# atx/padne

Measured on AMD Instinct MI355X. Metric: CG solves/s, higher is better.
Workload: dtype f64; 1 GPU; C4 8-layer N=10M: 8-layer jittered triangular Laplacian, 9999392 nodes, via-ring stitched, 1 A source/sink, amg-PCG to rtol 1e-12; n_unknowns=9999391, nnz_per_rank=69955225, rows_per_rank=9999391, parallelism=layer-partitioned x1

## Files before the change

padne_amd/_hip.py:

```python
from __future__ import annotations

import ctypes as C
import weakref
import os
import sys
from dataclasses import dataclass

import numpy as np

_HERE = os.path.dirname(os.path.abspath(__file__))
LIB_PATH = os.path.join(_HERE, "libpadne_hip.so")

OK = 0
E_INVALID, E_HIP, E_NOMEM, E_NONMANIFOLD, E_NOTCONVERGED, E_COMM, E_BREAKDOWN, E_TOOLARGE, E_NOCOARSEN = \
    -1, -2, -3, -4, -5, -6, -7, -8, -9


class HipUnavailableError(RuntimeError):
    """libpadne_hip.so cannot be loaded or no MI355X is visible."""


class HipError(RuntimeError):
    def __init__(self, code: int, message: str):
        super().__init__(f"libpadne_hip error {code}: {message}")
# ... 80 lines not shown
                                            _PI64, _PF64, _I64, _PI64, _PF64, C.POINTER(SolveOpts), C.c_double,
                                            C.POINTER(SolveInfo)]),
    "padne_kkt_power_density_block": (C.c_int, [_P, _P, C.c_int32, _PF64]),
    "padne_kkt_sensitivity_block": (C.c_int, [_P, _P, C.c_int32, C.c_int32, _PF64, _PF64, _PF64, _PF64]),
    "padne_kkt_current_report": (C.c_int, [_P, _P, C.c_int32, C.c_int64, C.c_int32, _PI32, C.c_int32, _PI32, _PF64, _PF64, _PF64,
                                           _PF64, _PI64, _PF64]),
    "padne_kkt_current_cases": (C.c_int, [_P, _P, C.c_int32, C.c_int64, C.c_int32, _PI32, C.c_int32, _PI32, _PF64, _PF64, _PF64,
                                          _PF64, _PI32, _PF64, _PI64, _PF64, _PF64]),
    "padne_kkt_error_estimate": (C.c_int, [_P, _P, C.c_int32, C.c_int64, C.c_int64, C.c_int32, _PF64, _PF64, _PF64, _PF64, _PF64,
                                           _PI64]),
    "padne_amg_apply": (C.c_int, [_P, _P, _PF64, _PF64]),
    "padne_amg_apply_batch": (C.c_int, [_P, _P, C.c_int32, _PF64, _PF64, _PF64]),
    "padne_csr_set_preconditioner_block": (C.c_int, [_P, _P]),
    "padne_amg_level": (C.c_int, [_P, _P, C.c_int, C.c_int, C.POINTER(_P)]),
    "padne_nearest_vertex": (C.c_int, [_P, _I64, _PF64, _I64, _PF64, _PI64]),
    "padne_nearest_vertex_ties": (C.c_int, [_P, _I64, _PF64, _I64, _PF64, _PI64, _PI32]),
    "padne_power_density": (C.c_int, [_P, _I64, _PF64, _I64, _PI32, _I64, _PI64, _PI64, _PF64, _PF64, _PF64]),
    "padne_csr_power_density": (C.c_int, [_P, _P, _PF64, _PF64]),
    "padne_face_gradient": (C.c_int, [_P, _I64, _PF64, _I64, _PI32, _I64, _PI64, _PI64, _PF64, _PF64, _PF64]),
    "padne_error_estimate": (C.c_int, [_P, _I64, _PF64, _I64, _PI32, _I64, _PI64, _PI64, _PF64, _PF64, _PF64, _PF64, _PF64, _PF64,
                                       _PF64, _PI64]),
    "padne_refine_create": (C.c_int, [_P, _I64, _PF64, _I64, _PI32, _I64, _PI64, _PI64, C.POINTER(C.c_uint8), _PI64, _PI64, _PI64,
                                      C.POINTER(_P)]),
    "padne_refine_fetch": (C.c_int, [_P, _P, _PF64, _PI32, _PI32, _PI32]),
    "padne_refine_destroy": (C.c_int, [_P]),
    "padne_sampler_create": (C.c_int, [_P, _I64, _PF64, _I64, _PI32, C.c_int32, _PI64, _PI64, _PI32, _PF64, C.c_int32, _PF64, _I64,
                                       C.POINTER(_P)]),
    "padne_sampler_destroy": (C.c_int, [_P]),
    "padne_sampler_points": (C.c_int, [_P, _P, C.c_int32, _I64, _PF64, _PI32, _PF64, _PF64, _PF64]),
    "padne_sampler_raster": (C.c_int, [_P, _P, C.c_int32, C.c_double, C.c_double, C.c_double, C.c_double, _I64, _I64, _PI32,
                                       _PF64, _PF64, _PF64]),
    "padne_sampler_stats": (C.c_int, [_P, C.c_int32, _PI64, _PF64]),
    "padne_spmv_algorithmic_bytes": (_I64, [_P]),
    "padne_spmv_time": (C.c_int, [_P, _P, _P, _P, C.c_int, C.c_int, _PF64]),
}

TEST_SIGNATURES = {
    "padne_team_create": (C.c_int, [C.c_int, C.POINTER(_P)]),
    "padne_team_destroy": (C.c_int, [_P]),
    "padne_team_abort": (C.c_int, [_P]),
    "padne_ctx_join_team": (C.c_int, [_P, _P, C.c_int]),
    "padne_csr_split_tiles": (C.c_int, [_P, C.c_int, _PI64, _PI64]),
    "padne_ctx_lockstep_groups": (C.c_int, [_P, _PI64]),
    "padne_asm_second_path_count": (C.c_int, [_PI64]),
    "padne_ctx_halo_exchange_time": (C.c_int, [_P, C.c_int32, C.POINTER(C.c_double)]),
    "padne_ctx_reload_options": (C.c_int, [_P]),
}

PROBE_SIGNATURES = {
    "padne_test_product": (C.c_int, [_P, _P, C.c_int32, _I64, C.c_int32, C.c_int32, C.c_int32, C.c_int32, _P, _P, _P, _P, _P,
                                     _P, _P, _P, _P, C.c_double, _P, _PF64, _I64, _PI32]),
}

_lib = None


def load_library(path: str | None = None) -> C.CDLL:
    global _lib
    if _lib is not None and path is None:
        return _lib
    p = path or LIB_PATH
    if not os.path.exists(p):
        raise HipUnavailableError(
            f"{p} not found: build it with `python -m padne_amd.build` (hipcc --offload-arch=gfx950). "
            "padne_amd has no CPU fallback.")
    if "torch" in sys.modules:
        pass
    try:
        lib = C.CDLL(p, mode=C.RTLD_GLOBAL)
    except OSError as exc:
        raise HipUnavailableError(f"cannot load {p}: {exc}") from exc
    for name, (res, args) in list(SIGNATURES.items()) + list(TEST_SIGNATURES.items()) + list(PROBE_SIGNATURES.items()):
        fn = getattr(lib, name)
        fn.restype = res
        fn.argtypes = args
    if lib.padne_abi_version() != 1:
        raise HipUnavailableError("libpadne_hip.so ABI version mismatch; rebuild it")
    if path is None:
        _lib = lib
    return lib


def _check(rc: int) -> None:
    if rc == OK:
        return
    msg = (load_library().padne_last_error() or b"").decode("utf-8", "replace")
    if rc == E_NONMANIFOLD:
        raise ValueError(msg or "Non-manifold mesh")
    if rc == E_INVALID:
        raise ValueError(msg)
    if rc == E_NOMEM:
        raise MemoryError(msg)
    if rc == E_TOOLARGE:
        raise OverflowError(msg)
    if rc == E_NOTCONVERGED:
        raise NotConvergedError(rc, msg)
    raise HipError(rc, msg)


def _f64(a) -> np.ndarray:
    return np.ascontiguousarray(a, dtype=np.float64)


def _i32(a) -> np.ndarray:
    return np.ascontiguousarray(a, dtype=np.int32)


def _i64(a) -> np.ndarray:
    return np.ascontiguousarray(a, dtype=np.int64)


def _ptr(a: np.ndarray, typ):
    return a.ctypes.data_as(typ)


def device_count() -> int:
    n = load_library().padne_device_count()
    return max(n, 0)


def launch_count() -> int:
    n = C.c_longlong(0)
    _check(load_library().padne_launch_count(C.byref(n)))
    return int(n.value)

# ... 65 lines not shown
        _check(self._lib.padne_ctx_comm_init(self._h, buf, int(rank), int(world_size)))

    def comm_init_host(self, rank: int, world_size: int, allgather):
        world_size = int(world_size)

        def cb(_user, send, recv, nbytes):
            try:
                src = np.ctypeslib.as_array(C.cast(send, C.POINTER(C.c_ubyte)), shape=(int(nbytes),)).copy()
                out = np.frombuffer(allgather(src), dtype=np.uint8)
                if out.size != world_size * int(nbytes):
                    return 2
                C.memmove(recv, out.ctypes.data, out.size)
                return 0
            except BaseException:
                return 1
        self._host_allgather = ALLGATHER_FN(cb)
        _check(self._lib.padne_ctx_comm_init_host(self._h, int(rank), world_size, C.cast(self._host_allgather, _P), None))

    def p2p_export(self, slots_per_rank: int) -> bytes:
        buf = C.create_string_buffer(64)
        _check(self._lib.padne_ctx_p2p_export(self._h, int(slots_per_rank), buf))
        return buf.raw

    def p2p_import(self, handles: bytes, world_size: int) -> None:
        buf = C.create_string_buffer(bytes(handles), 64 * int(world_size))
        _check(self._lib.padne_ctx_p2p_import(self._h, buf, int(world_size)))

    def p2p_selftest(self) -> bool:
        ok = C.c_int32(0)
        _check(self._lib.padne_ctx_p2p_selftest(self._h, C.byref(ok)))
        return bool(ok.value)

    def p2p_close(self) -> None:
        _check(self._lib.padne_ctx_p2p_close(self._h))

    def comm_call_counts(self):
        calls = (C.c_longlong * 4)()
        nbytes = (C.c_longlong * 4)()
        _check(self._lib.padne_comm_call_counts(calls, nbytes))
        return list(calls), list(nbytes)

    def reload_options(self) -> None:
        _check(self._lib.padne_ctx_reload_options(self._h))

    def halo_exchange_time(self, repeats: int = 200) -> float:
        t = C.c_double(0.0)
        _check(self._lib.padne_ctx_halo_exchange_time(self._h, int(repeats), C.byref(t)))
        return float(t.value)

    def lockstep_groups(self) -> int:
        g = C.c_int64(0)
        _check(self._lib.padne_ctx_lockstep_groups(self._h, C.byref(g)))
        return int(g.value)

    def set_halo(self, n_owned: int, m: int, export_idx) -> None:
        e = _i32(export_idx)
        _check(self._lib.padne_ctx_set_halo(self._h, int(n_owned), int(m), int(e.shape[0]), _ptr(e, _PI32)))
        self.halo_n_owned = int(n_owned)

    def clear_halo(self) -> None:
        _check(self._lib.padne_ctx_set_halo(self._h, -1, 0, 0, None))
        self.halo_n_owned = None

    def alloc(self, nbytes: int) -> int:
        p = _P()
        _check(self._lib.padne_dev_alloc(self._h, int(nbytes), C.byref(p)))
        return int(p.value)

    def free(self, dev: int):
        _check(self._lib.padne_dev_free(self._h, _P(dev)))

    def upload(self, dev: int, host: np.ndarray):
        host = np.ascontiguousarray(host)
        _check(self._lib.padne_dev_upload(self._h, _P(dev), host.ctypes.data_as(_P), host.nbytes))

    def download(self, dev: int, shape, dtype=np.float64) -> np.ndarray:
        out = np.empty(shape, dtype=dtype)
        _check(self._lib.padne_dev_download(self._h, out.ctypes.data_as(_P), _P(dev), out.nbytes))
        return out

    def to_device(self, host: np.ndarray) -> "DeviceArray":
        host = np.ascontiguousarray(host)
        d = DeviceArray(self, host.shape, host.dtype)
        self.upload(d.ptr, host)
        return d

    def empty(self, shape, dtype=np.float64) -> "DeviceArray":
        return DeviceArray(self, shape, dtype)

    def csr_from_scipy(self, A) -> "CsrMatrix":
        import scipy.sparse as sp
        A = sp.csr_matrix(A)
        A.sum_duplicates()
        A.sort_indices()
        if A.nnz >= 2**31 - 8192:
            raise ValueError("matrix too large for int32 indices")
        indptr, indices, data = _i32(A.indptr), _i32(A.indices), _f64(A.data)
        h = _P()
        _check(self._lib.padne_csr_from_host(self._h, A.shape[0], A.shape[1], _ptr(indptr, _PI32),
                                             _ptr(indices, _PI32), _ptr(data, _PF64), C.byref(h)))
        return CsrMatrix(self, h)

    def assemble_system(self, n_unknowns, xy, tri, mesh_vertex_offset, mesh_tri_offset, conductance,
                        coo_row, coo_col, coo_val, partial_mesh: bool = False) -> "CsrMatrix":
        xy_dev = isinstance(xy, DeviceArray)
        tri_dev = isinstance(tri, DeviceArray)
# ... 695 lines not shown
```

padne_amd/build.py:

```python
from __future__ import annotations

import os
import shutil
import subprocess
import sys

HERE = os.path.dirname(os.path.abspath(__file__))
CSRC = os.path.join(HERE, "csrc")
LIB = os.path.join(HERE, "libpadne_hip.so")
SOURCES = ["capi.hip", "spmv.hip", "spmm.hip", "pcg.hip", "assemble.hip", "comm.hip", "amg.hip", "generate.hip", "kkt.hip", "sample.hip", "error.hip", "refine.hip"]
HEADERS = ["common.hpp", "face.hpp", os.path.join("..", "..", "include", "padne_hip.h"),
           os.path.join("..", "..", "include", "padne_hip_test.h"), os.path.join("..", "..", "include", "padne_hip_probe.h")]
ARCH = "gfx950"
FLAGS = ["-O3", "-std=c++17", "-fPIC", f"--offload-arch={ARCH}", "-ffp-contract=off",
         "-fno-fast-math", "-Wall", "-Wno-unused-function", "-Wno-unused-value", "-Wno-unused-result"]


def hipcc() -> str:
    exe = shutil.which("hipcc") or "/opt/rocm/bin/hipcc"
    if not os.path.exists(exe):
        raise RuntimeError("hipcc not found: libpadne_hip.so cannot be built")
    return exe


def needs_build() -> bool:
    if not os.path.exists(LIB):
        return True
    t = os.path.getmtime(LIB)
    deps = [os.path.join(CSRC, s) for s in SOURCES + HEADERS] + [os.path.abspath(__file__)]
    return any(os.path.getmtime(d) > t for d in deps)


def build(force: bool = False, verbose: bool = True) -> str:
    if not force and not needs_build():
        return LIB
    objs = []
    cc = hipcc()
    os.makedirs(os.path.join(CSRC, "build"), exist_ok=True)
    procs = []
    for src in SOURCES:
        obj = os.path.join(CSRC, "build", src.replace(".hip", ".o"))
        cmd = [cc, *FLAGS, "-c", os.path.join(CSRC, src), "-o", obj]
        if verbose:
            print(" ".join(cmd), flush=True)
        procs.append((src, subprocess.Popen(cmd)))
        objs.append(obj)
    for src, p in procs:
        if p.wait() != 0:
            raise RuntimeError(f"hipcc failed on {src}")
    cmd = [cc, "-shared", "-fPIC", f"--offload-arch={ARCH}", "-o", LIB, *objs, "-ldl",
           "-Wl,-rpath,/opt/rocm/lib"]
    if verbose:
        print(" ".join(cmd), flush=True)
    subprocess.check_call(cmd)
    return LIB


if __name__ == "__main__":
    build(force="--force" in sys.argv)
    print(LIB)
```

padne_amd/csrc/assemble.hip:

```cpp
#include "common.hpp"
#include "face.hpp"

#include <atomic>

#include <cmath>

#include <algorithm>

#include <string.h>

namespace padne {

constexpr int kScanItems = 16;
constexpr int kScanChunk = 256 * kScanItems;

__device__ __forceinline__ int block_exclusive_scan_256(int v, int *lds , int *total) {
    const int lane = threadIdx.x & 63, w = threadIdx.x >> 6;
    int inc = v;
#pragma unroll
    for (int off = 1; off < 64; off <<= 1) {
        const int t = __shfl_up(inc, off, 64);
        if (lane >= off) inc += t;
    }
    if (lane == 63) lds[w] = inc;
// ... 115 lines not shown
    }
    if (blockIdx.x == 0 && threadIdx.x == 0) out[n] = (int)(*total);
}

constexpr int kScanSmall = 32768;
__global__ __launch_bounds__(1024) void scan_small(const int *in, const int n, int *out,
                                                   long long *__restrict__ total_out, unsigned long long *mail_slot,
                                                   unsigned long long mail_seq) {
    __shared__ long long wave_tot[16];
    __shared__ int any_neg;
    const int t = threadIdx.x, lane = t & 63, w = t >> 6;
    if (t == 0) any_neg = 0;
    __syncthreads();
    const int per = (n + 1023) / 1024;
    const int b0 = min(t * per, n), b1 = min(b0 + per, n);
    long long s = 0;
    bool neg = false;
    for (int i = b0; i < b1; ++i) {
        const int v = in[i];
        neg |= v < 0;
        s += v;
    }
    if (neg) any_neg = 1;
    long long inc = s;
#pragma unroll
    for (int off = 1; off < 64; off <<= 1) {
        const long long u = __shfl_up(inc, off, 64);
        if (lane >= off) inc += u;
    }
    if (lane == 63) wave_tot[w] = inc;
    __syncthreads();
    long long run = inc - s, total = 0;
    for (int q = 0; q < 16; ++q) {
        if (q < w) run += wave_tot[q];
        total += wave_tot[q];
    }
    for (int i = b0; i < b1; ++i) {
        const int v = in[i];
        out[i] = (int)run;
        run += v;
    }
    if (t == 0) {
        const long long tot = any_neg ? 0 : total;
        out[n] = (int)tot;
        total_out[0] = tot;
        total_out[1] = any_neg;
        if (mail_slot != nullptr) {
            const unsigned long long wd[2] = {(unsigned long long)tot, (unsigned long long)any_neg};
            mail_post(mail_slot, mail_seq, wd, 2);
        }
    }
}

int scan_i32_begin(padne_ctx *ctx, const int32_t *in, int32_t *out, int64_t n, ScanTicket *t, bool want_total) {
    const int nb = (int)((n + kScanChunk - 1) / kScanChunk);
    hipStream_t s = ctx->stream;
    t->nb = nb;
    t->bs = nullptr;
    t->want_total = want_total;
    t->mail = MailTicket();
    if (nb == 0) {
        const hipError_t e = hipMemsetAsync(out, 0, sizeof(int32_t), s);
        if (e != hipSuccess) {
            set_error("scan failed: %s", hipGetErrorString(e));
            return PADNE_E_HIP;
        }
        return PADNE_OK;
    }
    long long *bs = (long long *)pool_alloc(ctx, sizeof(long long) * (size_t)(nb + 2));
    if (bs == nullptr) return PADNE_E_NOMEM;
    t->bs = bs;
    long long *tot = bs + nb;
    if (want_total) t->mail = mail_ticket(ctx);
    if (n <= kScanSmall) {
        hipLaunchKernelGGL(scan_small, dim3(1), dim3(1024), 0, s, in, (int)n, out, tot, t->mail.slot_dev, t->mail.seq);
    } else {
        hipLaunchKernelGGL(scan_block_sums, dim3(nb), dim3(256), 0, s, in, (long long)n, bs);
        hipLaunchKernelGGL(scan_block_offsets, dim3(1), dim3(256), 0, s, bs, nb, tot, t->mail.slot_dev, t->mail.seq);
        hipLaunchKernelGGL(scan_apply, dim3(nb), dim3(256), 0, s, in, (long long)n, bs, tot, out);
    }
    const hipError_t e = hipGetLastError();
    if (e != hipSuccess) {
        pool_free(ctx, bs);
        t->bs = nullptr;
        set_error("scan failed: %s", hipGetErrorString(e));
        return PADNE_E_HIP;
    }
    return PADNE_OK;
}

int scan_i32_end(padne_ctx *ctx, ScanTicket *t, long long h[2]) {
    h[0] = h[1] = 0;
    if (t->nb == 0) return PADNE_OK;
    hipStream_t s = ctx->stream;
    long long *tot = t->bs + t->nb;
    hipError_t e = hipSuccess;
    int rc = PADNE_OK;
    if (t->want_total) {
        if (t->mail.slot_dev != nullptr) {
            rc = mail_wait(ctx, t->mail, h, 2 * sizeof(long long));
        } else {
            e = hipMemcpyAsync(h, tot, 2 * sizeof(long long), hipMemcpyDeviceToHost, s);
            if (e == hipSuccess) e = hipStreamSynchronize(s);
        }
    }
    pool_free(ctx, t->bs);
    t->bs = nullptr;
    if (e != hipSuccess) {
        set_error("scan failed: %s", hipGetErrorString(e));
        return PADNE_E_HIP;
    }
    return rc;
}

static int scan_i32_impl(padne_ctx *ctx, const int32_t *in, int32_t *out, int64_t n, long long h[2], bool want_total) {
    ScanTicket t;
    PADNE_TRY(scan_i32_begin(ctx, in, out, n, &t, want_total));
    return scan_i32_end(ctx, &t, h);
}

int exclusive_scan_i32(padne_ctx *ctx, const int32_t *in, int32_t *out, int64_t n, int64_t *total) {
    long long h[2] = {0, 0};
    PADNE_TRY(scan_i32_impl(ctx, in, out, n, h, true));
    if (h[0] < 0 || h[1] != 0) {
        set_error("scan of negative counts");
        return PADNE_E_INVALID;
    }
    if (h[0] >= 2147483647LL) {
// ... 256 lines not shown
    const bool fc = hubs_of == nullptr || hubs_of[gc] > kIncCap;
    if (!(fa || fb || fc)) return;
    const double ax = xy[2 * (long long)ga], ay = xy[2 * (long long)ga + 1];
    const double bx = xy[2 * (long long)gb], by = xy[2 * (long long)gb + 1];
    const double cx = xy[2 * (long long)gc], cy = xy[2 * (long long)gc + 1];
    const double wab = cot_half(ax, ay, bx, by, cx, cy);
    const double wbc = cot_half(bx, by, cx, cy, ax, ay);
    const double wca = cot_half(cx, cy, ax, ay, bx, by);
    int s;
    if (fa) {
        s = slot_ptr[ga] + atomicAdd(&cursor[ga], 2);
        key[s] = make_key(gb, 0); val[s] = wab;
        key[s + 1] = make_key(gc, 1); val[s + 1] = wca;
    }
    if (fb) {
        s = slot_ptr[gb] + atomicAdd(&cursor[gb], 2);
        key[s] = make_key(gc, 0); val[s] = wbc;
        key[s + 1] = make_key(ga, 1); val[s + 1] = wab;
    }
    if (fc) {
        s = slot_ptr[gc] + atomicAdd(&cursor[gc], 2);
        key[s] = make_key(ga, 0); val[s] = wca;
        key[s + 1] = make_key(gb, 1); val[s + 1] = wbc;
    }
}

__global__ __launch_bounds__(256) void asm_fill_listed(const int *__restrict__ n_list, const int *__restrict__ row_list,
                                                       long long n_vert, const double *__restrict__ xy,
                                                       const int *__restrict__ n_inc, const int2 *__restrict__ inc,
                                                       const int *__restrict__ slot_ptr, int *__restrict__ cursor,
                                                       long long *__restrict__ key, double *__restrict__ val) {
    const int idx = blockIdx.x * blockDim.x + threadIdx.x;
    if (idx >= *n_list) return;
    const int r = row_list[idx];
    const int T = r < n_vert ? n_inc[r] : 0;
    if (T > kIncCap) {
        cursor[r] = 1;
        return;
    }
    cursor[r] = 1 + 2 * T;
    if (T == 0) return;
    const double2 pv = reinterpret_cast<const double2 *>(xy)[r];
    const int s0 = slot_ptr[r];
    for (int q = 0; q < T; ++q) {
        const int2 jk = inc[inc_at(r, q, n_vert)];
        const double2 pj = reinterpret_cast<const double2 *>(xy)[jk.x], pk = reinterpret_cast<const double2 *>(xy)[jk.y];
        key[s0 + 1 + 2 * q] = make_key(jk.x, 0);
        val[s0 + 1 + 2 * q] = cot_half(pv.x, pv.y, pj.x, pj.y, pk.x, pk.y);
        key[s0 + 2 + 2 * q] = make_key(jk.y, 1);
        val[s0 + 2 + 2 * q] = cot_half(pk.x, pk.y, pv.x, pv.y, pj.x, pj.y);
    }
}

constexpr unsigned long long kScanValueMask = (1ull << 62) - 1ull;
constexpr unsigned long long kScanKnown = 1ull << 62;
constexpr int kScanMaxPolls = 1 << 20;
constexpr int kChunkTiles = 64;
__device__ __forceinline__ unsigned long long scan_word_load(const unsigned long long *p) {
    return __hip_atomic_load(p, __ATOMIC_RELAXED, __HIP_MEMORY_SCOPE_AGENT);
}
__device__ __forceinline__ void scan_word_store(unsigned long long *p, unsigned long long v) {
    __hip_atomic_store(p, v, __ATOMIC_RELAXED, __HIP_MEMORY_SCOPE_AGENT);
}
struct TileScan {
    unsigned long long *tile_agg;
    unsigned long long *chunk_agg;
    unsigned long long *chunk_prefix;
    int *chunk_count;
    int *ticket, *abort_word;
    long long *nnz_out;
    int n_tiles, n_chunks;
};

__device__ __forceinline__ void chunk_offset_scanner(const TileScan sc) {
    const int lane = threadIdx.x & 63;
    long long running = 0;
    int done = 0;
    if (lane == 0) scan_word_store(&sc.chunk_prefix[0], kScanKnown);
    int idle = 0;
    while (done < sc.n_chunks) {
        const int idx = done + lane;
        const unsigned long long w = idx < sc.n_chunks ? scan_word_load(&sc.chunk_agg[idx]) : 0ull;
        const unsigned long long gaps = __ballot((w >> 62) == 0ull);
        const int lead = gaps != 0ull ? __ffsll((long long)gaps) - 1 : 64;
        if (lead == 0) {
            if (++idle > kScanMaxPolls || ((idle & 255) == 0 && __hip_atomic_load(sc.abort_word, __ATOMIC_RELAXED, __HIP_MEMORY_SCOPE_AGENT) != 0)) {
                if (lane == 0) __hip_atomic_store(sc.abort_word, 1, __ATOMIC_RELAXED, __HIP_MEMORY_SCOPE_AGENT);
                return;
            }
            __builtin_amdgcn_s_sleep(2);
            continue;
        }
        idle = 0;
        long long incl = lane < lead ? (long long)(w & kScanValueMask) : 0;
        for (int off = 1; off < 64; off <<= 1) {
            const long long up = __shfl_up(incl, off, 64);
            if (lane >= off) incl += up;
        }
        if (lane < lead) scan_word_store(&sc.chunk_prefix[idx + 1], kScanKnown | (unsigned long long)(running + incl));
        running += __shfl(incl, 63, 64);
        done += lead;
    }
    if (lane == 0) *sc.nnz_out = running;
}

__device__ __forceinline__ int tile_publish(const TileScan sc, const int tile, const int total, const int lane) {
    int arrived = 0;
    if (lane == 0) {
        scan_word_store(&sc.tile_agg[tile], kScanKnown | (unsigned long long)total);
        arrived = __hip_atomic_fetch_add(&sc.chunk_count[tile / kChunkTiles], 1, __ATOMIC_RELAXED, __HIP_MEMORY_SCOPE_AGENT) + 1;
    }
    return arrived;
}
__device__ __forceinline__ bool chunk_publish(const TileScan sc, const int tile, const int arrived_lane0, const int lane) {
    const int c = tile / kChunkTiles;
    const int in_chunk = min(kChunkTiles, sc.n_tiles - c * kChunkTiles);
// ... 2220 lines not shown
                if (rc == PADNE_OK && e == hipSuccess) rc = read_back(ctx, d_err, sizeof(h_err), h_err);
            }
        }
        if (rc == PADNE_OK && e != hipSuccess) {
            set_error("row kernel failed: %s", hipGetErrorString(e));
            rc = PADNE_E_HIP;
        }
        if (rc == PADNE_OK && (h_err[ERR_SCAN] || h_err[ERR_GAVE_UP])) {
            set_error("the rows of the assembled system do not fit their offsets (inconsistent row lengths)");
            rc = PADNE_E_HIP;
        }
        if (rc == PADNE_OK && h_err[ERR_NONMANIFOLD] && !t_partial_mesh) {
            set_error("Non-manifold mesh");
            rc = PADNE_E_NONMANIFOLD;
        }
    } else {
        PADNE_HIP_CHECK(hipMemsetAsync(m->rowptr, 0, sizeof(int32_t), s));
    }
    if (rc == PADNE_OK && (h_nnz < 0 || h_nnz > nnz_bound)) {
        set_error("assembled %lld entries where at most %lld fit", h_nnz, nnz_bound);
        rc = PADNE_E_HIP;
    }
    if (rc == PADNE_OK) {
        rc = csr_shrink_nnz(ctx, m, h_nnz);
        if (rc == PADNE_OK && hipStreamSynchronize(s) != hipSuccess) {
            set_error("assembly failed: %s", hipGetErrorString(hipGetLastError()));
            rc = PADNE_E_HIP;
        }
    }
    if (rc != PADNE_OK) {
        padne_csr_destroy(m);
        return rc;
    }
    *out = m;
    padne_csr *res = *out;
    res->mesh_xy = keep_xy;
    res->mesh_tri = keep_tri;
    res->mesh_sigma = d_sigma;
    res->mesh_voff = d_voff;
    res->mesh_toff = d_toff;
    res->mesh_n_vert = n_vert;
    res->mesh_n_tri = n_tri;
    res->mesh_n_mesh = n_mesh;
    keep.released = true;
    return PADNE_OK;
}

extern "C" int padne_asm_second_path_count(int64_t *count) {
    PADNE_REQUIRE(count != nullptr, "count");
    *count = (int64_t)g_two_pass_fallbacks.load();
    return PADNE_OK;
}

extern "C" int padne_csr_power_density(padne_ctx *ctx, const padne_csr *m, const double *potential_host,
                                       double *power_out_host) {
    PADNE_REQUIRE(ctx && m, "null argument");
    PADNE_REQUIRE(m->mesh_n_mesh > 0 || m->mesh_n_tri == 0, "the matrix does not carry a mesh (only padne_assemble_system keeps it)");
    if (m->mesh_n_tri == 0) return PADNE_OK;
    PADNE_REQUIRE(potential_host && power_out_host, "null argument");
    PADNE_HIP_CHECK(hipSetDevice(ctx->device));
    hipStream_t s = ctx->stream;
    Scratch sc(ctx);
    double *d_pot = nullptr, *d_out = nullptr;
    int *d_bad = nullptr;
    PADNE_TRY(sc.alloc(&d_pot, (size_t)m->mesh_n_vert));
    PADNE_TRY(sc.alloc(&d_out, (size_t)m->mesh_n_tri));
    PADNE_TRY(sc.alloc(&d_bad, 1));
    PADNE_HIP_CHECK(hipMemsetAsync(d_bad, 0, sizeof(int), s));
    PADNE_HIP_CHECK(hipMemcpyAsync(d_pot, potential_host, sizeof(double) * (size_t)m->mesh_n_vert, hipMemcpyHostToDevice, s));
    hipLaunchKernelGGL(power_density_kernel, dim3(nblk(m->mesh_n_tri)), dim3(256), 0, s, (long long)m->mesh_n_tri, m->mesh_tri,
                       m->mesh_xy, (int)m->mesh_n_mesh, m->mesh_voff, m->mesh_toff, m->mesh_sigma, d_pot, d_out,
                       (double *)nullptr, (double *)nullptr, d_bad);
    PADNE_HIP_CHECK(hipGetLastError());
    PADNE_HIP_CHECK(hipMemcpyAsync(power_out_host, d_out, sizeof(double) * (size_t)m->mesh_n_tri, hipMemcpyDeviceToHost, s));
    PADNE_HIP_CHECK(hipStreamSynchronize(s));
    return PADNE_OK;
}

namespace padne {
int launch_power_density_block(padne_ctx *ctx, const padne_csr *m, int n_cols, const double *V_dev, double *out_dev,
                               int *bad_dev) {
    PADNE_REQUIRE(m->mesh_n_mesh > 0 && m->mesh_xy != nullptr, "the matrix does not carry a mesh (only padne_assemble_system keeps it)");
    if (m->mesh_n_tri == 0 || n_cols == 0) return PADNE_OK;
    hipLaunchKernelGGL(power_density_block_kernel, dim3(nblk(m->mesh_n_tri)), dim3(256), 0, ctx->stream, (long long)m->mesh_n_tri,
                       m->mesh_tri, m->mesh_xy, (int)m->mesh_n_mesh, m->mesh_voff, m->mesh_toff, m->mesh_sigma, n_cols, V_dev,
                       out_dev, bad_dev);
    PADNE_HIP_CHECK(hipGetLastError());
    return PADNE_OK;
}

int launch_sensitivity_block(padne_ctx *ctx, const padne_csr *m, const long long *tile_off_host, int n_cols, int n_obj,
                             const double *W_dev, const double *V_dev, double *power_dev, double *density_dev, double *total_dev,
                             int *bad_dev) {
    PADNE_REQUIRE(m->mesh_n_mesh > 0 && m->mesh_xy != nullptr, "the matrix does not carry a mesh (only padne_assemble_system keeps it)");
    const int n_mesh = (int)m->mesh_n_mesh;
    const long long n_blocks = tile_off_host[n_mesh];
    if (n_cols == 0 || n_obj == 0) return PADNE_OK;
    hipStream_t s = ctx->stream;
    Scratch sc(ctx);
    long long *d_tile = nullptr;
    double *d_partial = nullptr;
    PADNE_TRY(sc.alloc(&d_tile, (size_t)n_mesh + 1));
    PADNE_TRY(sc.alloc(&d_partial, (size_t)n_obj * (size_t)(n_blocks > 0 ? n_blocks : 1)));
    PADNE_HIP_CHECK(hipMemcpyAsync(d_tile, tile_off_host, sizeof(long long) * ((size_t)n_mesh + 1), hipMemcpyHostToDevice, s));
    if (n_blocks > 0) {
        hipLaunchKernelGGL(sensitivity_block_kernel, dim3((unsigned)n_blocks), dim3(256), 0, s, n_mesh, (const long long *)d_tile,
// ... 552 lines not shown
```

padne_amd/csrc/capi.hip:

```cpp
#include "common.hpp"

#include <algorithm>

#include <math.h>
#include <stdarg.h>
#include <string.h>
#include <chrono>

namespace padne {

std::atomic<long long> g_launch_count{0};

void options_from_env(padne_options *o) {
    *o = padne_options();
    auto on = [](const char *name) { const char *e = getenv(name); return e != nullptr && e[0] != '\0' && !(e[0] == '0' && e[1] == '\0'); };
    auto has = [](const char *list, const char *word) {
        const size_t n = strlen(word);
        for (const char *p = list; p != nullptr && *p != '\0';) {
            const char *q = strchr(p, ',');
            const size_t len = q != nullptr ? (size_t)(q - p) : strlen(p);
            if (len >= n && strncmp(p, word, n) == 0 && (len == n || p[n] == ':')) return p;
            p = q != nullptr ? q + 1 : nullptr;
        }
        return (const char *)nullptr;
    };
    o->amg_f64 = on("PADNE_AMG_F64");
    if (const char *e = getenv("PADNE_AMG_W")) o->amg_w = strcmp(e, "none") == 0 ? 0 : (strcmp(e, "fine") == 0 ? 1 : 2);
    o->amg_exchange_all = on("PADNE_AMG_EXCHANGE_ALL");
    o->pcg_p64 = on("PADNE_PCG_P64");
    o->pcg_no_xhist = on("PADNE_PCG_NO_XHIST");
    o->gj_vector = on("PADNE_GJ_VECTOR");
    o->no_batch = on("PADNE_NO_BATCH");
    o->no_mailbox = on("PADNE_NO_MAILBOX");
    o->no_p2p = on("PADNE_NO_P2P");
    o->no_split = on("PADNE_NO_SPLIT");
    o->no_xwindow = on("PADNE_NO_XWINDOW");
    o->setup_one_stream = on("PADNE_SETUP_ONE_STREAM");
    if (const char *e = getenv("PADNE_CG_SINGLE_REDUCTION")) o->cg_single_reduction = atoi(e) != 0 ? 1 : 0;
    if (const char *e = getenv("PADNE_LOCKSTEP_NARROW")) o->lockstep_narrow = atoi(e);
    if (const char *e = getenv("PADNE_AMG_COARSE_N")) o->amg_coarse_n = std::min(4096, std::max(16, atoi(e)));
    if (const char *e = getenv("PADNE_AMG_GATHER_N")) o->amg_gather_n = atoll(e);
    if (const char *e = getenv("PADNE_P2P_TIMEOUT_MS")) {
        const long v = atol(e);
        if (v > 0 && v <= 600000) o->p2p_timeout_ms = (unsigned)v;
    }
    if (const char *f = getenv("PADNE_FORCE")) {
        o->force_asm_hash = has(f, "asm_hash") != nullptr;
        o->force_asm_two_pass = has(f, "asm_two_pass") != nullptr;
        o->force_relabel_slots = has(f, "relabel_slots") != nullptr;
        o->force_transpose_cursors = has(f, "transpose_cursors") != nullptr;
        o->force_xhist_small = has(f, "xhist_small") != nullptr;
        o->force_relabel_lanes = has(f, "relabel_lanes") != nullptr;
        if (const char *w = has(f, "spgemm_split")) o->force_spgemm_split = w[12] == ':' ? atoll(w + 13) : 30000;
    }
    if (const char *v = getenv("PADNE_VERBOSE")) {
        o->verbose_amg = has(v, "amg") != nullptr;
        o->verbose_xw = has(v, "xw") != nullptr;
        o->verbose_pool = has(v, "pool") != nullptr;
    }
}

static thread_local char g_err[1024] = "";

void set_error(const char *fmt, ...) {
    va_list ap;
    va_start(ap, fmt);
    vsnprintf(g_err, sizeof(g_err), fmt, ap);
    va_end(ap);
}

int ensure_workspace(padne_ctx *ctx, size_t bytes) {
    if (ctx->ws_bytes >= bytes) return PADNE_OK;
    if (ctx->ws) {
        PADNE_HIP_CHECK(hipStreamSynchronize(ctx->stream));
        PADNE_HIP_CHECK(hipFree(ctx->ws));
        ctx->ws = nullptr;
        ctx->ws_bytes = 0;
    }
    if (hipMalloc(&ctx->ws, bytes) != hipSuccess) {
        set_error("hipMalloc of %zu workspace bytes failed", bytes);
        return PADNE_E_NOMEM;
    }
    ctx->ws_bytes = bytes;
    return PADNE_OK;
}

constexpr size_t kPoolCacheLimit = (size_t)240 << 30;

static size_t pool_round(size_t bytes) {
    if (bytes < 256) bytes = 256;
    if (bytes >= ((size_t)1 << 20)) return (bytes + ((size_t)1 << 20) - 1) & ~(((size_t)1 << 20) - 1);
    size_t p = 256;
    while (p < bytes) p <<= 1;
    return p;
}

void *pool_alloc(padne_ctx *ctx, size_t bytes) {
    const size_t want = pool_round(bytes);
    auto it = ctx->pool_free_blocks.lower_bound(want);
    if (it != ctx->pool_free_blocks.end() && it->first <= want + want / 2 + ((size_t)1 << 20)) {
        void *p = it->second;
        ctx->pool_cached_bytes -= it->first;
        ctx->pool_free_blocks.erase(it);
        return p;
    }
// ... 239 lines not shown

extern "C" {

int padne_abi_version(void) { return PADNE_ABI_VERSION; }

const char *padne_last_error(void) { return g_err; }

int padne_device_count(void) {
    int n = 0;
    hipError_t e = hipGetDeviceCount(&n);
    if (e != hipSuccess) {
        set_error("hipGetDeviceCount: %s", hipGetErrorString(e));
        return PADNE_E_HIP;
    }
    return n;
}

int padne_ctx_create(int device, padne_ctx **out) {
    PADNE_REQUIRE(out != nullptr, "out");
    int n = 0;
    PADNE_HIP_CHECK(hipGetDeviceCount(&n));
    if (n <= 0) {
        set_error("no HIP device visible: libpadne_hip has no CPU fallback");
        return PADNE_E_HIP;
    }
    PADNE_REQUIRE(device >= 0 && device < n, "device index out of range");
    PADNE_HIP_CHECK(hipSetDevice(device));
    padne_ctx *ctx = new padne_ctx();
    ctx->device = device;
    options_from_env(&ctx->opt);
    ctx->p2p_timeout_ms = ctx->opt.p2p_timeout_ms;
    if (ctx_init_resources(ctx) != PADNE_OK) {
        padne_ctx_destroy(ctx);
        return PADNE_E_HIP;
    }
    *out = ctx;
    return PADNE_OK;
}

int padne_ctx_destroy(padne_ctx *ctx) {
    if (!ctx) return PADNE_OK;
    hipSetDevice(ctx->device);
    if (ctx->stream) hipStreamSynchronize(ctx->stream);
    if (ctx->aux) {
        padne_ctx_destroy(ctx->aux);
        ctx->aux = nullptr;
    }
    comm_destroy(ctx);
    pool_release_all(ctx);
    for (auto &kv : ctx->pool_sizes) (void)hipFree(kv.first);
    ctx->pool_sizes.clear();
    if (ctx->halo_export) hipFree(ctx->halo_export);
    if (ctx->ws) hipFree(ctx->ws);
    if (ctx->partials) hipFree(ctx->partials);
    if (ctx->scalars) hipFree(ctx->scalars);
    if (ctx->status) hipFree(ctx->status);
    if (ctx->pinned) hipHostFree(ctx->pinned);
    if (ctx->mailbox) hipHostFree(ctx->mailbox);
    if (ctx->ev0) hipEventDestroy(ctx->ev0);
    if (ctx->ev1) hipEventDestroy(ctx->ev1);
    if (ctx->ev_order) hipEventDestroy(ctx->ev_order);
    for (hipStream_t &cs : ctx->copy_stream)
        if (cs != nullptr) {
            (void)hipStreamSynchronize(cs);
            (void)hipStreamDestroy(cs);
            cs = nullptr;
        }
    if (ctx->stream) hipStreamDestroy(ctx->stream);
    delete ctx;
    return PADNE_OK;
}

int padne_ctx_synchronize(padne_ctx *ctx) {
    PADNE_REQUIRE(ctx, "ctx");
    PADNE_HIP_CHECK(hipStreamSynchronize(ctx->stream));
    return PADNE_OK;
}

void *padne_ctx_stream(padne_ctx *ctx) { return ctx ? (void *)ctx->stream : nullptr; }

int padne_dev_alloc(padne_ctx *ctx, int64_t bytes, void **dev_out) {
    PADNE_REQUIRE(ctx && dev_out && bytes >= 0, "arguments");
    PADNE_HIP_CHECK(hipSetDevice(ctx->device));
    if (hipMalloc(dev_out, bytes > 0 ? (size_t)bytes : 8) != hipSuccess) {
        set_error("hipMalloc(%lld) failed", (long long)bytes);
        return PADNE_E_NOMEM;
    }
    return PADNE_OK;
}

int padne_dev_free(padne_ctx *ctx, void *dev) {
    PADNE_REQUIRE(ctx, "ctx");
    if (dev) {
        PADNE_HIP_CHECK(hipStreamSynchronize(ctx->stream));
        PADNE_HIP_CHECK(hipFree(dev));
    }
    return PADNE_OK;
}

int padne_dev_upload(padne_ctx *ctx, void *dev_dst, const void *host_src, int64_t bytes) {
    PADNE_REQUIRE(ctx && bytes >= 0 && (bytes == 0 || (dev_dst && host_src)), "arguments");
    if (bytes == 0) return PADNE_OK;
    PADNE_HIP_CHECK(hipMemcpyAsync(dev_dst, host_src, (size_t)bytes, hipMemcpyHostToDevice, ctx->stream));
    PADNE_HIP_CHECK(hipStreamSynchronize(ctx->stream));
    return PADNE_OK;
}
// ... 182 lines not shown
```

padne_amd/csrc/common.hpp:

```cpp
#pragma once

#include <hip/hip_runtime.h>
#include <stdint.h>
#include <stdio.h>
#include <map>
#include <string>
#include <unordered_map>
#include <vector>

#include "../../include/padne_hip.h"
#include "../../include/padne_hip_test.h"
#include "../../include/padne_hip_probe.h"

#include <atomic>

namespace padne {

extern std::atomic<long long> g_launch_count;

void set_error(const char *fmt, ...);

#define PADNE_HIP_CHECK(expr)                                                              \
    do {                                                                                   \
        hipError_t _e = (expr);                                                            \
        if (_e != hipSuccess) {                                                            \
            ::padne::set_error("%s failed: %s (%s:%d)", #expr, hipGetErrorString(_e),      \
                               __FILE__, __LINE__);                                        \
            return PADNE_E_HIP;                                                            \
        }                                                                                  \
    } while (0)

#define PADNE_REQUIRE(cond, msg)                                                           \
    do {                                                                                   \
        if (!(cond)) {                                                                     \
            ::padne::set_error("invalid argument: %s (%s)", msg, #cond);                   \
            return PADNE_E_INVALID;                                                        \
        }                                                                                  \
    } while (0)

#define PADNE_TRY(...)                                                                     \
    do {                                                                                   \
        int _rc = (__VA_ARGS__);                                                           \
        if (_rc != PADNE_OK) return _rc;                                                   \
    } while (0)

}
#undef hipLaunchKernelGGL
#define hipLaunchKernelGGL(kernelName, numBlocks, numThreads, memPerBlock, streamId, ...)   \
    do {                                                                                   \
        ::padne::g_launch_count.fetch_add(1, std::memory_order_relaxed);                   \
        kernelName<<<(numBlocks), (numThreads), (memPerBlock), (streamId)>>>(__VA_ARGS__); \
    } while (0)
#define hipMemsetAsync(...) (::padne::g_launch_count.fetch_add(1, std::memory_order_relaxed), hipMemsetAsync(__VA_ARGS__))
namespace padne {

constexpr int kNumXcd = 8;

constexpr int kSpmvThreads = 256;
constexpr int kSpmvRows = 256;
constexpr int kPadNnz = 4096;

constexpr int kMaxPartials = 2048;
constexpr int kPinnedSlots = 16;
constexpr int kPinnedSlotBase = 4096;
constexpr int kPinnedBytes = kPinnedSlotBase + 512 * kPinnedSlots;
// ... 2 lines not shown
constexpr int kSpmmK = 8;

}

struct padne_csr {
    int64_t n_rows = 0, n_cols = 0, nnz = 0;
    int32_t *rowptr = nullptr;
    int32_t *cols = nullptr;
    double *vals = nullptr;
    double *dinv = nullptr;
    int device = 0;
    padne_ctx *owner = nullptr;
    void *amg = nullptr;
    float *vals32 = nullptr, *dinv32 = nullptr;
    int4 *xw_desc = nullptr;
    unsigned short *xw_lidx = nullptr;
    int xw_state = 0;
    int xw_run = 0;
    int xw_nruns = 3;
    int *split_tiles = nullptr;
    int split_n_int = 0, split_n_bnd = 0;
    int split_state = 0;
    bool hierarchy_operator = false;
    bool cols_unsorted = false;
    padne_csr *prec_block = nullptr;
    double *mesh_xy = nullptr, *mesh_sigma = nullptr;
    int32_t *mesh_tri = nullptr;
    long long *mesh_voff = nullptr, *mesh_toff = nullptr;
    int64_t mesh_n_vert = 0, mesh_n_tri = 0, mesh_n_mesh = 0;
};

struct padne_options {
    bool amg_f64 = false;
    int amg_w = 2;
    bool amg_exchange_all = false;
    bool pcg_p64 = false;
    bool pcg_no_xhist = false;
    bool gj_vector = false;
    bool no_batch = false;
    bool no_mailbox = false;
    bool no_p2p = false;
    bool no_split = false;
    bool no_xwindow = false;
    bool setup_one_stream = false;
    int cg_single_reduction = -1;
    int lockstep_narrow = -1;
    int amg_coarse_n = 2048;
    long long amg_gather_n = 0;
    unsigned p2p_timeout_ms = 20000;
    bool force_asm_hash = false, force_asm_two_pass = false, force_relabel_slots = false, force_transpose_cursors = false;
    bool force_relabel_lanes = false;
    bool force_xhist_small = false;
    long long force_spgemm_split = 0;
    bool verbose_amg = false, verbose_xw = false, verbose_pool = false;
};
namespace padne { void options_from_env(padne_options *o); }

struct padne_ctx {
    int device = 0;
    padne_options opt;
    hipStream_t stream = nullptr;
    double *partials = nullptr;
    double *scalars = nullptr;
    int32_t *status = nullptr;
    void *pinned = nullptr;
    void *ws = nullptr;
    size_t ws_bytes = 0;
    void *comm = nullptr;
    void *team = nullptr;
    int rank = 0, world = 1;
    bool halo_on = false;
    long long halo_n_owned = 0;
    int halo_m = 0, halo_n_export = 0;
    int32_t *halo_export = nullptr;
    void *p2p_mbox = nullptr;
    void **p2p_peers = nullptr;
    int p2p_m_cap = 0;
    unsigned long long p2p_seq = 0;
    bool p2p_ipc = false;
    std::vector<void *> p2p_ipc_mapped;
    unsigned p2p_timeout_ms = 20000;
    int (*hostcoll_fn)(void *, const void *, void *, int64_t) = nullptr;
    void *hostcoll_user = nullptr;
    hipEvent_t ev0 = nullptr, ev1 = nullptr;
    hipStream_t copy_stream[4] = {nullptr, nullptr, nullptr, nullptr};
    padne_ctx *aux = nullptr, *parent = nullptr;
    bool is_aux = false;
    unsigned long long lockstep_groups = 0;
    unsigned pinned_busy = 0;
    unsigned long long *mailbox = nullptr, *mailbox_dev = nullptr;
    unsigned long long mail_seq = 0;
    hipEvent_t ev_order = nullptr;
    std::multimap<size_t, void *> pool_free_blocks;
    std::unordered_map<void *, size_t> pool_sizes;
    size_t pool_cached_bytes = 0;
};

namespace padne {

int ensure_workspace(padne_ctx *ctx, size_t bytes);
int csr_alloc(padne_ctx *ctx, int64_t n_rows, int64_t n_cols, int64_t nnz, padne_csr **out);
int csr_shrink_nnz(padne_ctx *ctx, padne_csr *m, int64_t nnz);
int csr_build_dinv(padne_ctx *ctx, padne_csr *m);

int spmv_grid(const padne_csr *m);
enum { SPMV_PLAIN = 0, SPMV_DOT = 1, SPMV_RESID = 2, SPMV_ADD = 3, SPMV_JACOBI = 4,
       SPMV_DOT_AUX = 5,
       SPMV_WUP = 6,
       SPMV_RESTRICT = 7,
       SPMV_RESID_PRE = 8 };
enum { SPMV_ALL = 0, SPMV_INTERIOR = 1, SPMV_BOUNDARY = 2 };

template <typename XT> struct ProductArgs {
    const XT *b = nullptr;
    const XT *dinv = nullptr;
    XT scale = 0;
    const XT *x_pre = nullptr;
    XT *y2 = nullptr;
    const XT *rhs = nullptr;
    const double *dot_with = nullptr;
// ... 141 lines not shown
```

Baseline: 31.68 solves/s.

## Replace three-pass int32 exclusive scan with single-pass decoupled look-back scan

Large int32 exclusive scans now use one kernel that takes a tile ticket, publishes each tile's aggregate and inclusive prefix in global status words, and looks back across predecessors, in place of the block-sums, block-offsets and apply kernels. This removes two launches and a second pass over the input. If a tile exceeds its poll budget it gives up, and the last block redoes those tiles serially. The status words persist in the context and are reset by the last block. Scans are used in setup and assembly rather than in the CG iteration, so the effect on solve throughput is probably small.

```diff
diff --git a/padne_amd/_hip.py b/padne_amd/_hip.py
--- a/padne_amd/_hip.py
+++ b/padne_amd/_hip.py
@@ -156,6 +156,11 @@
                                      _P, _P, _P, _P, C.c_double, _P, _PF64, _I64, _PI32]),
 }
 
+SCAN_TEST_SIGNATURES = {
+    "padne_test_exclusive_scan_i32": (C.c_int, [_P, _P, _P, _I64, C.c_int32, _PI64, _PI32]),
+    "padne_ctx_scan_fallback_count": (C.c_int, [_P, _PI64]),
+}
+
 _lib = None
 
 
@@ -174,7 +179,7 @@
         lib = C.CDLL(p, mode=C.RTLD_GLOBAL)
     except OSError as exc:
         raise HipUnavailableError(f"cannot load {p}: {exc}") from exc
-    for name, (res, args) in list(SIGNATURES.items()) + list(TEST_SIGNATURES.items()) + list(PROBE_SIGNATURES.items()):
+    for name, (res, args) in list(SIGNATURES.items()) + list(TEST_SIGNATURES.items()) + list(PROBE_SIGNATURES.items()) + list(SCAN_TEST_SIGNATURES.items()):
         fn = getattr(lib, name)
         fn.restype = res
         fn.argtypes = args
@@ -346,6 +351,18 @@
         g = C.c_int64(0)
         _check(self._lib.padne_ctx_lockstep_groups(self._h, C.byref(g)))
         return int(g.value)
+
+    def exclusive_scan_i32(self, src: "DeviceArray", dst: "DeviceArray", n: int, form: str = "total"):
+        total = C.c_int64(-1)
+        neg = C.c_int32(0)
+        rc = self._lib.padne_test_exclusive_scan_i32(self._h, _P(src.ptr), _P(dst.ptr), int(n),
+                                                     {"total": 0, "async": 1, "flagged": 2}[form], C.byref(total), C.byref(neg))
+        return int(rc), int(total.value), bool(neg.value)
+
+    def scan_fallback_count(self) -> int:
+        n = C.c_int64(0)
+        _check(self._lib.padne_ctx_scan_fallback_count(self._h, C.byref(n)))
+        return int(n.value)
 
     def set_halo(self, n_owned: int, m: int, export_idx) -> None:
         e = _i32(export_idx)
diff --git a/padne_amd/build.py b/padne_amd/build.py
--- a/padne_amd/build.py
+++ b/padne_amd/build.py
@@ -10,7 +10,8 @@
 LIB = os.path.join(HERE, "libpadne_hip.so")
 SOURCES = ["capi.hip", "spmv.hip", "spmm.hip", "pcg.hip", "assemble.hip", "comm.hip", "amg.hip", "generate.hip", "kkt.hip", "sample.hip", "error.hip", "refine.hip"]
 HEADERS = ["common.hpp", "face.hpp", os.path.join("..", "..", "include", "padne_hip.h"),
-           os.path.join("..", "..", "include", "padne_hip_test.h"), os.path.join("..", "..", "include", "padne_hip_probe.h")]
+           os.path.join("..", "..", "include", "padne_hip_test.h"), os.path.join("..", "..", "include", "padne_hip_probe.h"),
+           os.path.join("..", "..", "include", "padne_hip_scan_test.h")]
 ARCH = "gfx950"
 FLAGS = ["-O3", "-std=c++17", "-fPIC", f"--offload-arch={ARCH}", "-ffp-contract=off",
          "-fno-fast-math", "-Wall", "-Wno-unused-function", "-Wno-unused-value", "-Wno-unused-result"]
diff --git a/padne_amd/csrc/assemble.hip b/padne_amd/csrc/assemble.hip
--- a/padne_amd/csrc/assemble.hip
+++ b/padne_amd/csrc/assemble.hip
@@ -191,6 +191,197 @@
     }
 }
 
+constexpr unsigned long long kScanValueMask = (1ull << 62) - 1ull;
+constexpr unsigned long long kScanKnown = 1ull << 62;
+constexpr unsigned long long kScanPrefix = 1ull << 63;
+constexpr unsigned long long kScanNegBit = 1ull << 61;
+constexpr unsigned long long kScanSumMask = (1ull << 61) - 1ull;
+constexpr int kScanMaxPolls = 1 << 20;
+enum { kScanCtlTicket = 0, kScanCtlDone = 1, kScanCtlGaveUp = 2, kScanCtlFallbacks = 3, kScanCtlWords = 16 };
+__device__ __forceinline__ unsigned long long scan_word_load(const unsigned long long *p) {
+    return __hip_atomic_load(p, __ATOMIC_RELAXED, __HIP_MEMORY_SCOPE_AGENT);
+}
+__device__ __forceinline__ void scan_word_store(unsigned long long *p, unsigned long long v) {
+    __hip_atomic_store(p, v, __ATOMIC_RELAXED, __HIP_MEMORY_SCOPE_AGENT);
+}
+
+__device__ __forceinline__ void scan_tile_load(const int *in, long long n, long long chunk, bool vec, int (&v)[kScanItems]) {
+#pragma unroll
+    for (int j = 0; j < kScanItems / 4; ++j) {
+        const long long e = chunk + ((long long)j * 256 + threadIdx.x) * 4;
+        if (vec && e + 3 < n) {
+            const int4 q = *reinterpret_cast<const int4 *>(in + e);
+            v[4 * j] = q.x; v[4 * j + 1] = q.y; v[4 * j + 2] = q.z; v[4 * j + 3] = q.w;
+        } else {
+#pragma unroll
+            for (int t = 0; t < 4; ++t) v[4 * j + t] = e + t < n ? in[e + t] : 0;
+        }
+    }
+}
+__device__ __forceinline__ void scan_tile_write(int *out, long long n, long long chunk, bool vec, const int (&v)[kScanItems],
+                                                int carry, int *lds ) {
+#pragma unroll
+    for (int j = 0; j < kScanItems / 4; ++j) {
+        const long long e = chunk + ((long long)j * 256 + threadIdx.x) * 4;
+        const int v0 = v[4 * j], v1 = v[4 * j + 1], v2 = v[4 * j + 2];
+        int slab_total = 0;
+        const int run = carry + block_exclusive_scan_256(v0 + v1 + v2 + v[4 * j + 3], lds, &slab_total);
+        if (vec && e + 3 < n) {
+            *reinterpret_cast<int4 *>(out + e) = make_int4(run, run + v0, run + v0 + v1, run + v0 + v1 + v2);
+        } else {
+            if (e < n) out[e] = run;
+            if (e + 1 < n) out[e + 1] = run + v0;
+            if (e + 2 < n) out[e + 2] = run + v0 + v1;
+            if (e + 3 < n) out[e + 3] = run + v0 + v1 + v2;
+        }
+        carry += slab_total;
+    }
+}
+__device__ __forceinline__ void scan_post_total(int *out, long long n, long long total, bool any_neg, long long *total_out,
+                                                unsigned long long *mail_slot, unsigned long long mail_seq) {
+    out[n] = (int)total;
+    total_out[0] = total;
+    total_out[1] = any_neg;
+    if (mail_slot != nullptr) {
+        const unsigned long long w[2] = {(unsigned long long)total, (unsigned long long)any_neg};
+        mail_post(mail_slot, mail_seq, w, 2);
+    }
+}
+
+__global__ __launch_bounds__(256) void scan_chained(const int *in, const long long n, const int nb, int *out,
+                                                    unsigned long long *words , int *ctl ,
+                                                    long long *total_out, unsigned long long *mail_slot,
+                                                    const unsigned long long mail_seq, const int max_polls) {
+    __shared__ int lds[5];
+    __shared__ long long red[4];
+    __shared__ long long s_excl;
+    __shared__ int s_neg, s_tile, s_ok, s_last;
+    const int lane = threadIdx.x & 63, wv = threadIdx.x >> 6;
+    if (threadIdx.x == 0) {
+        s_tile = __hip_atomic_fetch_add(&ctl[kScanCtlTicket], 1, __ATOMIC_RELAXED, __HIP_MEMORY_SCOPE_AGENT);
+        s_neg = 0;
+        s_ok = 1;
+        s_excl = 0;
+    }
+    __syncthreads();
+    const int tile = s_tile;
+    const long long chunk = (long long)tile * kScanChunk;
+    const bool vec = ((reinterpret_cast<unsigned long long>(in) | reinterpret_cast<unsigned long long>(out)) & 15ull) == 0ull;
+    int v[kScanItems];
+    scan_tile_load(in, n, chunk, vec, v);
+    long long s = 0;
+    int ored = 0;
+#pragma unroll
+    for (int k = 0; k < kScanItems; ++k) {
+        s += v[k];
+        ored |= v[k];
+    }
+    for (int off = 32; off > 0; off >>= 1) s += __shfl_down(s, off, 64);
+    if (lane == 0) red[wv] = s;
+    if (ored < 0) s_neg = 1;
+    __syncthreads();
+    if (wv == 0) {
+        const bool own_neg = s_neg != 0;
+        const long long agg = own_neg ? 0 : (red[0] + red[1]) + (red[2] + red[3]);
+        const unsigned long long own = (own_neg ? kScanNegBit : 0ull) | ((unsigned long long)agg & kScanSumMask);
+        long long excl = 0;
+        bool neg_before = false, ok = true;
+        if (tile == 0) {
+            if (lane == 0) scan_word_store(&words[0], kScanPrefix | own);
+        } else {
+            if (lane == 0) scan_word_store(&words[tile], kScanKnown | own);
+            ok = max_polls > 0;
+            int polls = 0;
+            for (int base = tile - 1; ok; base -= 64) {
+                const int idx = base - lane;
+                unsigned long long w = idx >= 0 ? scan_word_load(&words[idx]) : kScanPrefix;
+                while (__any((w >> 62) == 0ull)) {
+                    if (++polls > max_polls) {
+                        ok = false;
+                        break;
+                    }
+                    if ((w >> 62) == 0ull) w = scan_word_load(&words[idx]);
+                }
+                if (!ok) break;
+                const unsigned long long has_prefix = __ballot((w & kScanPrefix) != 0ull);
+                const int first = has_prefix != 0ull ? __ffsll((long long)has_prefix) - 1 : 63;
+                long long part = lane <= first ? (long long)(w & kScanSumMask) : 0;
+                neg_before |= __any(lane <= first && (w & kScanNegBit) != 0ull) != 0;
+                for (int off = 32; off > 0; off >>= 1) part += __shfl_xor(part, off, 64);
+                excl += part;
+                if (has_prefix != 0ull) break;
+            }
+            if (lane == 0) {
+                if (ok) {
+                    const bool neg_incl = neg_before || own_neg;
+                    scan_word_store(&words[tile], kScanPrefix | (neg_incl ? kScanNegBit : 0ull) | ((unsigned long long)(excl + agg) & kScanSumMask));
+                } else {
+                    __hip_atomic_fetch_add(&ctl[kScanCtlGaveUp], 1, __ATOMIC_RELAXED, __HIP_MEMORY_SCOPE_AGENT);
+                }
+            }
+        }
+        if (lane == 0) {
+            s_ok = ok;
+            s_excl = excl;
+            if (ok && tile == nb - 1) scan_post_total(out, n, excl + agg, neg_before || own_neg, total_out, mail_slot, mail_seq);
+        }
+    }
+    __syncthreads();
+    if (s_ok) scan_tile_write(out, n, chunk, vec, v, (int)s_excl, lds);
+    __syncthreads();
+    if (threadIdx.x == 0) {
+        __builtin_amdgcn_fence(__ATOMIC_RELEASE, "workgroup");
+        s_last = __hip_atomic_fetch_add(&ctl[kScanCtlDone], 1, __ATOMIC_RELAXED, __HIP_MEMORY_SCOPE_AGENT) == nb - 1;
+    }
+    __syncthreads();
+    if (!s_last) return;
+    if (__hip_atomic_load(&ctl[kScanCtlGaveUp], __ATOMIC_RELAXED, __HIP_MEMORY_SCOPE_AGENT) != 0) {
+        long long run = 0;
+        bool any_neg = false;
+        for (int i = 0; i < nb; ++i) {
+            const unsigned long long w = scan_word_load(&words[i]);
+            if ((w & kScanPrefix) != 0ull) {
+                run = (long long)(w & kScanSumMask);
+                any_neg |= (w & kScanNegBit) != 0ull;
+                continue;
+            }
+            const long long c = (long long)i * kScanChunk;
+            scan_tile_load(in, n, c, vec, v);
+            scan_tile_write(out, n, c, vec, v, (int)run, lds);
+            run += (long long)(w & kScanSumMask);
+            any_neg |= (w & kScanNegBit) != 0ull;
+            if (i == nb - 1 && threadIdx.x == 0) scan_post_total(out, n, run, any_neg, total_out, mail_slot, mail_seq);
+        }
+        if (threadIdx.x == 0) ctl[kScanCtlFallbacks] += 1;
+    }
+    for (int i = threadIdx.x; i < nb; i += 256) scan_word_store(&words[i], 0ull);
+    if (threadIdx.x == 0) {
+        ctl[kScanCtlTicket] = 0;
+        ctl[kScanCtlDone] = 0;
+        ctl[kScanCtlGaveUp] = 0;
+    }
+}
+
+static int scan_state_reserve(padne_ctx *ctx, int nb) {
+    if (ctx->scan_state != nullptr && ctx->scan_state_tiles >= nb) return PADNE_OK;
+    if (ctx->scan_state != nullptr) {
+        PADNE_HIP_CHECK(hipStreamSynchronize(ctx->stream));
+        PADNE_HIP_CHECK(hipFree(ctx->scan_state));
+        ctx->scan_state = nullptr;
+        ctx->scan_state_tiles = 0;
+    }
+    const int tiles = std::max(nb, 1 << 14);
+    const size_t bytes = sizeof(unsigned long long) * (size_t)(kScanCtlWords / 2 + tiles);
+    if (hipMalloc(&ctx->scan_state, bytes) != hipSuccess) {
+        (void)hipGetLastError();
+        set_error("hipMalloc of %zu bytes of scan state failed", bytes);
+        return PADNE_E_NOMEM;
+    }
+    PADNE_HIP_CHECK(hipMemsetAsync(ctx->scan_state, 0, bytes, ctx->stream));
+    ctx->scan_state_tiles = tiles;
+    return PADNE_OK;
+}
+
 int scan_i32_begin(padne_ctx *ctx, const int32_t *in, int32_t *out, int64_t n, ScanTicket *t, bool want_total) {
     const int nb = (int)((n + kScanChunk - 1) / kScanChunk);
     hipStream_t s = ctx->stream;
@@ -206,6 +397,8 @@
         }
         return PADNE_OK;
     }
+    const bool chained = n > kScanSmall && !ctx->opt.force_scan_three_pass;
+    if (chained) PADNE_TRY(scan_state_reserve(ctx, nb));
     long long *bs = (long long *)pool_alloc(ctx, sizeof(long long) * (size_t)(nb + 2));
     if (bs == nullptr) return PADNE_E_NOMEM;
     t->bs = bs;
@@ -213,6 +406,11 @@
     if (want_total) t->mail = mail_ticket(ctx);
     if (n <= kScanSmall) {
         hipLaunchKernelGGL(scan_small, dim3(1), dim3(1024), 0, s, in, (int)n, out, tot, t->mail.slot_dev, t->mail.seq);
+    } else if (chained) {
+        int *ctl = (int *)ctx->scan_state;
+        hipLaunchKernelGGL(scan_chained, dim3(nb), dim3(256), 0, s, in, (long long)n, nb, out,
+                           (unsigned long long *)(ctl + kScanCtlWords), ctl, tot, t->mail.slot_dev, t->mail.seq,
+                           ctx->opt.force_scan_poll_budget0 ? 0 : kScanMaxPolls);
     } else {
         hipLaunchKernelGGL(scan_block_sums, dim3(nb), dim3(256), 0, s, in, (long long)n, bs);
         hipLaunchKernelGGL(scan_block_offsets, dim3(1), dim3(256), 0, s, bs, nb, tot, t->mail.slot_dev, t->mail.seq);
@@ -575,16 +773,7 @@
     }
 }
 
-constexpr unsigned long long kScanValueMask = (1ull << 62) - 1ull;
-constexpr unsigned long long kScanKnown = 1ull << 62;
-constexpr int kScanMaxPolls = 1 << 20;
 constexpr int kChunkTiles = 64;
-__device__ __forceinline__ unsigned long long scan_word_load(const unsigned long long *p) {
-    return __hip_atomic_load(p, __ATOMIC_RELAXED, __HIP_MEMORY_SCOPE_AGENT);
-}
-__device__ __forceinline__ void scan_word_store(unsigned long long *p, unsigned long long v) {
-    __hip_atomic_store(p, v, __ATOMIC_RELAXED, __HIP_MEMORY_SCOPE_AGENT);
-}
 struct TileScan {
     unsigned long long *tile_agg;
     unsigned long long *chunk_agg;
@@ -2911,6 +3100,39 @@
     return PADNE_OK;
 }
 
+extern "C" int padne_test_exclusive_scan_i32(padne_ctx *ctx, const int32_t *in_dev, int32_t *out_dev, int64_t n, int32_t form,
+                                             int64_t *total_out, int32_t *negative_out) {
+    PADNE_REQUIRE(ctx && out_dev && (n == 0 || in_dev) && total_out && negative_out, "null argument");
+    PADNE_REQUIRE(n >= 0 && n < 2147483647LL && form >= 0 && form <= 2, "arguments");
+    PADNE_HIP_CHECK(hipSetDevice(ctx->device));
+    *total_out = -1;
+    *negative_out = 0;
+    int rc = PADNE_OK;
+    if (form == 0) {
+        rc = exclusive_scan_i32(ctx, in_dev, out_dev, n, total_out);
+    } else if (form == 1) {
+        rc = exclusive_scan_i32_async(ctx, in_dev, out_dev, n);
+    } else {
+        bool negative = false;
+        rc = exclusive_scan_i32_flagged(ctx, in_dev, out_dev, n, total_out, &negative);
+        *negative_out = negative ? 1 : 0;
+    }
+    if (hipStreamSynchronize(ctx->stream) != hipSuccess && rc == PADNE_OK) rc = PADNE_E_HIP;
+    return rc;
+}
+
+extern "C" int padne_ctx_scan_fallback_count(padne_ctx *ctx, int64_t *count) {
+    PADNE_REQUIRE(ctx && count, "null argument");
+    *count = 0;
+    if (ctx->scan_state == nullptr) return PADNE_OK;
+    int h = 0;
+    PADNE_HIP_CHECK(hipSetDevice(ctx->device));
+    PADNE_HIP_CHECK(hipMemcpyAsync(&h, (const int *)ctx->scan_state + kScanCtlFallbacks, sizeof(int), hipMemcpyDeviceToHost, ctx->stream));
+    PADNE_HIP_CHECK(hipStreamSynchronize(ctx->stream));
+    *count = h;
+    return PADNE_OK;
+}
+
 extern "C" int padne_csr_power_density(padne_ctx *ctx, const padne_csr *m, const double *potential_host,
                                        double *power_out_host) {
     PADNE_REQUIRE(ctx && m, "null argument");
diff --git a/padne_amd/csrc/capi.hip b/padne_amd/csrc/capi.hip
--- a/padne_amd/csrc/capi.hip
+++ b/padne_amd/csrc/capi.hip
@@ -51,6 +51,8 @@
         o->force_transpose_cursors = has(f, "transpose_cursors") != nullptr;
         o->force_xhist_small = has(f, "xhist_small") != nullptr;
         o->force_relabel_lanes = has(f, "relabel_lanes") != nullptr;
+        o->force_scan_three_pass = has(f, "scan_three_pass") != nullptr;
+        o->force_scan_poll_budget0 = has(f, "scan_poll_budget0") != nullptr;
         if (const char *w = has(f, "spgemm_split")) o->force_spgemm_split = w[12] == ':' ? atoll(w + 13) : 30000;
     }
     if (const char *v = getenv("PADNE_VERBOSE")) {
@@ -396,6 +398,7 @@
     ctx->pool_sizes.clear();
     if (ctx->halo_export) hipFree(ctx->halo_export);
     if (ctx->ws) hipFree(ctx->ws);
+    if (ctx->scan_state) hipFree(ctx->scan_state);
     if (ctx->partials) hipFree(ctx->partials);
     if (ctx->scalars) hipFree(ctx->scalars);
     if (ctx->status) hipFree(ctx->status);
diff --git a/padne_amd/csrc/common.hpp b/padne_amd/csrc/common.hpp
--- a/padne_amd/csrc/common.hpp
+++ b/padne_amd/csrc/common.hpp
@@ -11,6 +11,7 @@
 #include "../../include/padne_hip.h"
 #include "../../include/padne_hip_test.h"
 #include "../../include/padne_hip_probe.h"
+#include "../../include/padne_hip_scan_test.h"
 
 #include <atomic>
 
@@ -119,6 +120,8 @@
     bool force_relabel_lanes = false;
     bool force_xhist_small = false;
     long long force_spgemm_split = 0;
+    bool force_scan_three_pass = false;
+    bool force_scan_poll_budget0 = false;
     bool verbose_amg = false, verbose_xw = false, verbose_pool = false;
 };
 namespace padne { void options_from_env(padne_options *o); }
@@ -133,6 +136,8 @@
     void *pinned = nullptr;
     void *ws = nullptr;
     size_t ws_bytes = 0;
+    void *scan_state = nullptr;
+    int scan_state_tiles = 0;
     void *comm = nullptr;
     void *team = nullptr;
     int rank = 0, world = 1;
```

Result: no change. 31.52 solves/s (-0.5%).
